# amathislab/BUCTD

Hardware: AMD Instinct MI355X
Metric: images/sec (train) BUCTD-CoAM-W48 384x288 (higher is better)
Workload: dtype f32 (3x3 convs: operands split exactly into 3 bf16 pieces, 6 bf16 MFMAs per product, fp32 accumulate - fp32-class); 1 GPU; BUCTD-CoAM-W48 (pose_hrnet_coam, ATT_MODULES [F,T,F,F], colored condition) 384x288 CrowdPose-14kpt full train step: fwd + JointsMSE + bwd + grad all-reduce + Adam + arg-max accuracy decode; global_batch=32, batch_per_gpu=32, input=N x 6 x 384 x 288 fp32, params=115581770, parallelism=dp1, hip_streams=4, conv_math=bf16x6, step_graph=False

## Files before the change

### buctd_amd/_C.py

```python
import ctypes as C
import os

import torch

_HERE = os.path.dirname(os.path.abspath(__file__))
LIB_PATH = os.path.join(_HERE, "lib", "libbuctd_hip.so")


class ConvDesc(C.Structure):
    _fields_ = [(n, C.c_int) for n in ("N", "H", "W", "Ci", "Co", "R", "S", "stride", "pad", "Ho", "Wo")]


class BasicBlockDesc(C.Structure):
    _fields_ = ([(n, C.c_int) for n in ("N", "H", "W", "C")] +
                [(n, C.c_void_p) for n in ("x", "w1_fwd", "w2_fwd", "w1_bwd", "w2_bwd", "gamma1", "beta1", "gamma2", "beta2",
                                           "running_mean1", "running_var1", "running_mean2", "running_var2")] +
                [(n, C.c_float) for n in ("eps1", "momentum1", "eps2", "momentum2")] +
                [(n, C.c_void_p) for n in ("z1", "z2", "y", "acc", "stat")])


class BasicBlockGrads(C.Structure):
    _fields_ = ([(n, C.c_void_p) for n in ("dy", "dz2", "dres", "dy1", "dz1", "dx", "dw1", "dw2", "dgamma1", "dbeta1",
                                           "dgamma2", "dbeta2")] +
                [(n, C.c_int) for n in ("acc_w1", "acc_w2", "acc_bn1", "acc_bn2")] +
# ... 2 lines not shown

class BnAccIn(C.Structure):
    _fields_ = [("acc", C.c_void_p), ("rows", C.c_long), ("eps", C.c_float), ("momentum", C.c_float),
                ("mean_out", C.c_void_p), ("invstd_out", C.c_void_p), ("running_mean", C.c_void_p),
                ("running_var", C.c_void_p)]


class C3Conv(C.Structure):
    _fields_ = ([(n, C.c_int) for n in ("N", "H", "W", "Ci", "Co")] +
                [(n, C.c_void_p) for n in ("x", "wprep", "residual")] + [("relu", C.c_int)] +
                [(n, C.c_void_p) for n in ("y", "stats_acc")] + [("in_bn", C.POINTER(BnAccIn))] +
                [(n, C.c_void_p) for n in ("in_gamma", "in_beta")] + [("in_relu", C.c_int)] +
                [(n, C.c_void_p) for n in ("bn_z", "bn_y", "bn_mean", "bn_invstd", "bn_gamma", "bn_beta", "bn_acc")])


class C3ConvEval(C.Structure):
    _fields_ = ([(n, C.c_int) for n in ("N", "H", "W", "Ci", "Co")] +
                [(n, C.c_void_p) for n in ("x", "wprep", "scale", "shift", "residual")] + [("relu", C.c_int), ("y", C.c_void_p)])


class BnApplyItem(C.Structure):
    _fields_ = [("z", C.c_void_p), ("st", BnAccIn), ("gamma", C.c_void_p), ("beta", C.c_void_p), ("residual", C.c_void_p),
                ("relu", C.c_int), ("y", C.c_void_p), ("rows", C.c_long), ("C", C.c_int)]


class BnBwdItem(C.Structure):
    _fields_ = ([(n, C.c_void_p) for n in ("dy", "y", "z", "mean", "invstd", "gamma", "beta")] +
                [("relu", C.c_int), ("rows", C.c_long), ("C", C.c_int)] +
                [(n, C.c_void_p) for n in ("dz", "dres", "dgamma", "dbeta")] +
                [("accumulate", C.c_int), ("acc", C.c_void_p), ("acc_ready", C.c_int)])


class Wg3Conv(C.Structure):
    _fields_ = ([(n, C.c_int) for n in ("N", "H", "W", "Ci", "Co")] +
                [(n, C.c_void_p) for n in ("x", "dy", "dw")] + [("accumulate", C.c_int)] +
                [(n, C.c_void_p) for n in ("x_mean", "x_invstd", "x_gamma", "x_beta")] + [("x_relu", C.c_int)] +
                [("workspace", C.c_void_p), ("workspace_bytes", C.c_size_t)])


class MhaArgs(C.Structure):
    _fields_ = ([(n, C.c_int) for n in ("B", "T", "h", "dh")] +
                [(n, C.c_void_p) for n in ("q", "k", "v")] + [(n, C.c_int) for n in ("ldq", "ldk", "ldv")] +
                [("out", C.c_void_p), ("ldo", C.c_int), ("lse", C.c_void_p), ("scale", C.c_float), ("p_drop", C.c_float),
                 ("dout", C.c_void_p), ("lddo", C.c_int)] +
                [(n, C.c_void_p) for n in ("dq", "dk", "dv")] + [(n, C.c_int) for n in ("lddq", "lddk", "lddv")])

# ... 108 lines not shown
    "buctd_conv3x3_wgrad_bf16x6_group_workgroups": (_I, [_I, C.POINTER(Wg3Conv)]),
    "buctd_stream_fork": (_I, [_P, _P]),
    "buctd_basic_branches_fwd_train": (_I, [_I, _I, C.POINTER(BasicBlockDesc), _P]),
    "buctd_basic_branches_bwd": (_I, [_I, _I, C.POINTER(BasicBlockDesc), C.POINTER(BasicBlockGrads), _P, _P]),
    "buctd_basic_chain_fwd_train": (_I, [_I, C.POINTER(BasicBlockDesc), _P]),
    "buctd_basic_chain_bwd": (_I, [_I, C.POINTER(BasicBlockDesc), C.POINTER(BasicBlockGrads), _P, _P]),
    "buctd_x6_image_dims": (_I, [_I, _I, _I, _P, _P]),
    "buctd_x6_image_bytes": (C.c_size_t, [_I, _I, _I]),
    "buctd_x6_image": (_I, [_P, _I, _I, _I, _L, _L, _I, _L, _L, _I, _P, _P]),
    "buctd_x6_gemm": (_I, [_I, _I, _I, _P, _P, _P, _I, _F, _P, _L, _I, _L, _P]),
    "buctd_add": (_I, [_P, _P, _P, _L, _I, _P]),
    "buctd_add_n": (_I, [C.POINTER(_P), _I, _P, _L, _P]),
    "buctd_mul": (_I, [_P, _P, _P, _L, _P]),
    "buctd_scale": (_I, [_P, _P, _F, _P, _L, _P]),
    "buctd_copy_channels": (_I, [_P, _L, _I, _I, _P, _I, _I, _I, _P]),
    "buctd_add_bcast": (_I, [_P, _P, _P, _L, _L, _P]),
    "buctd_relu_bwd": (_I, [_P, _P, _P, _L, _P]),
    "buctd_colsum_workspace": (_SZ, [_L, _I]),
    "buctd_colsum": (_I, [_P, _L, _I, _P, _I, _P, _SZ, _P]),
    "buctd_nchw_to_nhwc": (_I, [_P, _I, _I, _I, _I, _I, _I, _P, _P]),
    "buctd_nhwc_to_nchw": (_I, [_P, _I, _I, _I, _I, _P, _P]),
    "buctd_fuse_sum": (_I, [C.POINTER(_P), _PI, _I, _I, _I, _I, _I, _I, _P, _P]),
    "buctd_fuse_sum_bwd": (_I, [_P, _P, _I, _I, _I, _I, _I, _P, _P]),
    "buctd_resize_bilinear": (_I, [_P, _I, _I, _I, _I, _I, _I, _I, _I, _P, _P]),
    "buctd_maxpool3x3s2_fwd": (_I, [_P, _I, _I, _I, _I, _P, _P, _P]),
    "buctd_maxpool3x3s2_bwd": (_I, [_P, _P, _I, _I, _I, _I, _P, _P]),
    "buctd_softmax_dropout_fwd": (_I, [_P, _L, _I, _F, _F, _U64, _P, _P, _P]),
    "buctd_softmax_dropout_bwd": (_I, [_P, _P, _L, _I, _F, _F, _U64, _P, _P]),
    "buctd_softmax_dropout_fwd_dseed": (_I, [_P, _L, _I, _F, _F, _P, _P, _P, _P]),
    "buctd_softmax_dropout_bwd_dseed": (_I, [_P, _P, _L, _I, _F, _F, _P, _P, _P]),
    "buctd_dropout": (_I, [_P, _P, _L, _F, _U64, _P]),
    "buctd_dropout_dseed": (_I, [_P, _P, _L, _F, _P, _P]),
    "buctd_dropout_seed_fill": (_I, [_P, _I, _U64, _U64, _P]),
    "buctd_attn_smallqk_supported": (_I, [_I, _I, _I]),
    "buctd_attn_smallqk_fwd": (_I, [_I, _I, _I, _I, _P, _P, _P, _F, _F, _U64, _I, _P, _P, _P, _P]),
    "buctd_attn_smallqk_bwd": (_I, [_I, _I, _I, _I, _P, _P, _P, _P, _P, _P, _P, _F, _F, _U64, _I, _P, _P, _P, _P, _P]),
    "buctd_attn_smallqk_fwd_dseed": (_I, [_I, _I, _I, _I, _P, _P, _P, _F, _F, _P, _I, _P, _P, _P, _P]),
    "buctd_attn_smallqk_bwd_dseed": (_I, [_I, _I, _I, _I, _P, _P, _P, _P, _P, _P, _P, _F, _F, _P, _I, _P, _P, _P, _P, _P]),
    "buctd_layernorm_fwd": (_I, [_P, _P, _P, _L, _I, _F, _P, _P, _P, _P]),
    "buctd_add_layernorm_fwd": (_I, [_P, _P, _P, _P, _L, _I, _F, _P, _P, _P, _P, _P]),
    "buctd_layernorm_bwd_workspace": (_SZ, [_L, _I]),
    "buctd_layernorm_bwd": (_I, [_P, _P, _P, _P, _P, _L, _I, _P, _P, _P, _I, _P, _SZ, _P]),
    "buctd_joints_mse": (_I, [_P, _P, _P, _I, _I, _I, _P, _P, _F, _P, _SZ, _P]),
    "buctd_joints_ohkm_mse_workspace": (_SZ, [_I, _I]),
    "buctd_joints_ohkm_mse": (_I, [_P, _P, _P, _I, _I, _I, _I, _P, _P, _F, _P, _SZ, _P]),
    "buctd_argmax_decode": (_I, [_P, _I, _I, _I, _P, _P, _P, _P]),
# ... 102 lines not shown
```

### buctd_amd/csrc/bn.hip

```cpp
#include "common.h"
#include "../../include/buctd_hip.h"
#include "bn_acc.h"

#define STAT_ROWS 64

__global__ __launch_bounds__(256) void bn_stats_kernel(const float* __restrict__ z, long rows, int C,
                                                       float* __restrict__ part) {
  const long r0 = (long)blockIdx.x * STAT_ROWS;
  long r1 = r0 + STAT_ROWS;
  if (r1 > rows) r1 = rows;
  const int cnt = (int)(r1 - r0);
  for (int c = threadIdx.x; c < C; c += 256) {
    float s = 0.f;
    for (long r = r0; r < r1; ++r) s += z[r * C + c];
    const float mean = cnt > 0 ? s / (float)cnt : 0.f;
    float m2 = 0.f;
    for (long r = r0; r < r1; ++r) {
      const float d = z[r * C + c] - mean;
      m2 += d * d;
    }
    part[((long)blockIdx.x * C + c) * 2 + 0] = mean;
    part[((long)blockIdx.x * C + c) * 2 + 1] = m2;
  }
}

// ... 480 lines not shown
  const long total = rows * C;
  const float inv_rows = 1.0f / (float)rows;
  if (C % 4 == 0)
    hipLaunchKernelGGL(bn_bwd_apply_kernel<true>, dim3(stream_grid(total / 4)), dim3(256), 0, st, dy, y, z, mean,
                       invstd, gamma, beta, (const float*)s, relu, total, C, inv_rows, dz, dres);
  else
    hipLaunchKernelGGL(bn_bwd_apply_kernel<false>, dim3(stream_grid(total)), dim3(256), 0, st, dy, y, z, mean, invstd,
                       gamma, beta, (const float*)s, relu, total, C, inv_rows, dz, dres);
  BUCTD_CHECK_LAUNCH("buctd_bn_bwd_from_partials(apply)");
  return BUCTD_OK;
}

extern "C" int buctd_bn_fold(const float* gamma, const float* beta, const float* running_mean,
                             const float* running_var, float eps, int C, float* scale, float* shift, void* stream) {
  BUCTD_CHECK_ARG(gamma && beta && running_mean && running_var && scale && shift && C > 0,
                  "buctd_bn_fold: bad argument");
  hipLaunchKernelGGL(bn_fold_kernel, dim3(ceil_div(C, 256)), dim3(256), 0, (hipStream_t)stream, gamma, beta,
                     running_mean, running_var, eps, C, scale, shift);
  BUCTD_CHECK_LAUNCH("buctd_bn_fold");
  return BUCTD_OK;
}


#define BWD2_MAX_BLOCKS 1024

__global__ __launch_bounds__(256) void bn_bwd_reduce2_kernel(const float* __restrict__ dy, const float* __restrict__ y,
                                                             const float* __restrict__ z, const float* __restrict__ mean,
                                                             const float* __restrict__ invstd,
                                                             const float* __restrict__ gamma, const float* __restrict__ beta,
                                                             int relu, long rows, int C, long rows_per_block,
                                                             float* __restrict__ part) {
  __shared__ f32x4 sm[2][256];
  const int c4n = C >> 2;
  const int rl = 256 / c4n;
  const int tc = threadIdx.x % c4n, tr = threadIdx.x / c4n;
  const long r0 = (long)blockIdx.x * rows_per_block;
  long r1 = r0 + rows_per_block;
  if (r1 > rows) r1 = rows;
  f32x4 s1 = (f32x4){0.f, 0.f, 0.f, 0.f}, s2 = s1;
  if (tr < rl) {
    const f32x4 mu = reinterpret_cast<const f32x4*>(mean)[tc];
    const f32x4 is = reinterpret_cast<const f32x4*>(invstd)[tc];
    f32x4 sc = is, be = is;
    const bool rebuild = relu && !y;
    if (rebuild) {
      sc = is * reinterpret_cast<const f32x4*>(gamma)[tc];
      be = reinterpret_cast<const f32x4*>(beta)[tc];
    }
// ... 20 lines not shown
      }
#pragma unroll
      for (int u = 0; u < 4; ++u) body(g[u], zz[u], yy[u]);
    }
    for (; r < r1; r += step) {
      const long o = r * c4n + tc;
      const f32x4 zz = reinterpret_cast<const f32x4*>(z)[o];
      body(reinterpret_cast<const f32x4*>(dy)[o], zz, (relu && y) ? reinterpret_cast<const f32x4*>(y)[o] : zz);
    }
  }
  sm[0][threadIdx.x] = s1;
  sm[1][threadIdx.x] = s2;
  __syncthreads();
  if (tr == 0) {
    for (int k = 1; k < rl; ++k) {
      s1 += sm[0][k * c4n + tc];
      s2 += sm[1][k * c4n + tc];
    }
    reinterpret_cast<f32x4*>(part + ((long)blockIdx.x * 2 + 0) * C)[tc] = s1;
    reinterpret_cast<f32x4*>(part + ((long)blockIdx.x * 2 + 1) * C)[tc] = s2;
  }
}

static long bwd2_blocks(long rows, long* rows_per_block) {
  long rpb = (rows + BWD2_MAX_BLOCKS - 1) / BWD2_MAX_BLOCKS;
  if (rpb < 64) rpb = 64;
  *rows_per_block = rpb;
  return (rows + rpb - 1) / rpb;
}


static int acc_grid(long n4, int per_cu = 8) {
  long b = (n4 + 256 * 4 - 1) / (256 * 4);
  if (b > 256 * per_cu) b = 256 * per_cu;
  if (b < 1) b = 1;
  return (int)b;
}

struct BnApplyArgs {
  const float* z;
  BnAccFwd a;
  const float* gamma;
  const float* beta;
  const float* res;
  int relu;
  float* y;
  long total;
  int C;
};
__device__ __forceinline__ void bn_apply_acc_body(const BnApplyArgs& p, unsigned bid, unsigned nblk, unsigned char* lds_raw) {
  const float* __restrict__ z = p.z;
  const float* __restrict__ res = p.res;
  float* __restrict__ y = p.y;
  const BnAccFwd& a = p.a;
  const int C = p.C, relu = p.relu;
  long long* wsum = reinterpret_cast<long long*>(lds_raw);
  float* tab = reinterpret_cast<float*>(lds_raw + (size_t)BNACC_WORDS * C * sizeof(long long));
  const long n4 = p.total >> 2;
  const long step = (long)nblk * 256;
  long i = (long)bid * 256 + threadIdx.x;
// ... 422 lines not shown
```

### buctd_amd/models/hrnet_common.py

```python
import logging
import os

import torch

from .. import nn
from .. import ops

BN_MOMENTUM = 0.1
logger = logging.getLogger(__name__)


def conv3x3(in_planes, out_planes, stride=1):
    return nn.Conv2d(in_planes, out_planes, kernel_size=3, stride=stride, padding=1, bias=False)


class BasicBlock(nn.Module):
    expansion = 1

    def __init__(self, inplanes, planes, stride=1, downsample=None):
        super().__init__()
        self.conv1 = conv3x3(inplanes, planes, stride)
        self.bn1 = nn.BatchNorm2d(planes, momentum=BN_MOMENTUM)
        self.relu = nn.ReLU(inplace=True)
        self.conv2 = conv3x3(planes, planes)
# ... 164 lines not shown
                       and m.bn1.running_mean is not None and m.bn2.running_mean is not None for m in br):
                return None
            chains.append([_block_params(m) for m in br])
        xs = [x[i] for i in range(self.num_branches)]
        if not ops.eval_branches_ok(xs, chains):
            return None
        return ops.basic_branches_eval(xs, chains)

    def forward(self, x):
        if self.num_branches == 1:
            return [self.branches[0](x[0])]
        xs = self._branches_grouped(x)
        if xs is None:
            xs = self._branches_grouped_eval(x)
        if xs is None:
            xs = ops.fork_join([lambda i=i: self.branches[i](x[i]) for i in range(self.num_branches)],
                               [x[i] for i in range(self.num_branches)])
        rows = list(enumerate(self.fuse_layers))
        fan = len(rows) > 1 and torch.is_grad_enabled() and any(t.requires_grad for t in xs)
        xr = [ops.FanOut.apply(xs[j], len(rows)) if fan and xs[j].is_cuda else [xs[j]] * len(rows)
              for j in range(self.num_branches)]

        def fuse_row(i, row):
            terms, shifts = [], []
            for j in range(self.num_branches):
                if j == i:
                    terms.append(xr[j][i])
                    shifts.append(0)
                elif j > i:
                    terms.append(row[j](xr[j][i]))
                    shifts.append(j - i)
                else:
                    terms.append(row[j](xr[j][i]))
                    shifts.append(0)
            return ops.FuseSum.apply(tuple(shifts), True, *terms)

        return ops.fork_join([lambda i=i, row=row: fuse_row(i, row) for i, row in rows], [xs for _ in rows], tag=1)


def make_transition_layer(pre, cur):
    layers = []
    for i in range(len(cur)):
        if i < len(pre):
            if cur[i] != pre[i]:
                layers.append(nn.ConvBN(nn.Conv2d(pre[i], cur[i], 3, 1, 1, bias=False), nn.BatchNorm2d(cur[i]),
                                        nn.ReLU(inplace=True)))
            else:
                layers.append(None)
        else:
            steps = []
            for j in range(i + 1 - len(pre)):
                cin = pre[-1]
                cout = cur[i] if j == i - len(pre) else cin
                steps.append(nn.ConvBN(nn.Conv2d(cin, cout, 3, 2, 1, bias=False), nn.BatchNorm2d(cout),
                                       nn.ReLU(inplace=True)))
            layers.append(nn.Chain(*steps))
    return nn.ModuleList(layers)

# ... 89 lines not shown
```

### buctd_amd/ops.py

```python
import ctypes as C
import math
import weakref

import torch

from . import _C
from ._C import ConvDesc, MatmulDesc, check, lib, ptr, stream_ptr

_capture = {"on": False, "events": set(), "allow_seeds": False, "seed_table": None, "seed_draws": 0}
_SEED_TABLE_SLOTS = 1024


def capturing():
    return _capture["on"]


def _new_event(stream=None):
    ev = torch.cuda.Event()
    ev.record(stream) if stream is not None else ev.record()
    if _capture["on"]:
        _capture["events"].add(id(ev))
        _capture.setdefault("keep", []).append(ev)
    return ev

# ... 1876 lines not shown
class FuseSum(torch.autograd.Function):

    @staticmethod
    def forward(ctx, shifts, relu, *terms):
        out = fuse_sum(list(terms), list(shifts), relu)
        ctx.shifts, ctx.relu = shifts, relu
        ctx.save_for_backward(out if relu else None)
        return out

    @staticmethod
    def backward(ctx, dy):
        (y,) = ctx.saved_tensors
        dy = _contig(dy)
        cache = {}
        grads = []
        for j, s in enumerate(ctx.shifts):
            if not ctx.needs_input_grad[2 + j]:
                grads.append(None)
                continue
            if s not in cache:
                cache[s] = fuse_sum_bwd(dy, y, s) if s > 0 or ctx.relu else dy
            grads.append(cache[s])
        return (None, None, *grads)


class AddN(torch.autograd.Function):

    @staticmethod
    def forward(ctx, a, b, c):
        out = add(a, b)
        if c is not None:
            out = add(out, c, out=out)
        ctx.n = 3 if c is not None else 2
        return out

    @staticmethod
    def backward(ctx, dy):
        return dy, dy, (dy if ctx.n == 3 else None)


def add_n(terms):
    acc = terms[0]
    k = 1
    while k < len(terms):
        group = [acc] + list(terms[k:k + 3])
        k += 3
# ... 391 lines not shown
```

### include/buctd_hip.h

```cpp
#ifndef BUCTD_HIP_H
#define BUCTD_HIP_H
#include <stddef.h>
#include <stdint.h>

#ifdef __cplusplus
extern "C" {
#endif

int buctd_version(void);
const char* buctd_last_error(void);

typedef struct {
  int N, H, W, Ci;
  int Co, R, S;
  int stride, pad;
  int Ho, Wo;
} buctd_conv_desc;

int buctd_conv2d_fwd_thin(const buctd_conv_desc* d);
int buctd_conv2d_fwd(const buctd_conv_desc* d, const float* x, const float* w, const float* bias,
                     const float* scale, const float* shift, const float* residual, int relu, float* y,
                     float* stats_partials, void* stream);
int buctd_conv2d_dgrad(const buctd_conv_desc* d, const float* dy, const float* w, const float* bias, float* dx,
                       float* stats_partials, void* stream);
// ... 167 lines not shown
  int acc_ready;
} buctd_bn_bwd_item;
int buctd_bn_bwd_acc_group(int n, const buctd_bn_bwd_item* items, void* stream);
int buctd_bn_fold(const float* gamma, const float* beta, const float* running_mean, const float* running_var,
                  float eps, int C, float* scale, float* shift, void* stream);

int buctd_add(const float* a, const float* b, float* out, long n, int relu, void* stream);
int buctd_add_n(const float* const* terms, int n, float* out, long count, void* stream);
int buctd_mul(const float* a, const float* b, float* out, long n, void* stream);
int buctd_scale(const float* x, const float* dev_scalar, float alpha, float* out, long n, void* stream);
int buctd_copy_channels(const float* src, long rows, int Cs, int cs0, float* dst, int Cd, int cd0, int Cc,
                        void* stream);
int buctd_add_bcast(const float* a, const float* v, float* out, long batch, long n, void* stream);
int buctd_relu_bwd(const float* dy, const float* y, float* dx, long n, void* stream);
size_t buctd_colsum_workspace(long rows, int C);
int buctd_colsum(const float* x, long rows, int C, float* out, int accumulate, void* workspace,
                 size_t workspace_bytes, void* stream);
int buctd_nchw_to_nhwc(const float* x, int N, int Ctot, int c0, int Cc, int H, int W, float* y, void* stream);
int buctd_nhwc_to_nchw(const float* x, int N, int C, int H, int W, float* y, void* stream);
int buctd_fuse_sum(const float* const* terms, const int* shifts, int nterms, int N, int H, int W, int C, int relu,
                   float* out, void* stream);
int buctd_fuse_sum_bwd(const float* dy, const float* y, int shift, int N, int H, int W, int C, float* g,
                       void* stream);
int buctd_resize_bilinear(const float* x, int N, int Ctot, int c0, int Cc, int H, int W, int Ho, int Wo, float* y,
                          void* stream);
int buctd_maxpool3x3s2_fwd(const float* x, int N, int H, int W, int C, float* y, int32_t* idx, void* stream);
int buctd_maxpool3x3s2_bwd(const float* dy, const int32_t* idx, int N, int H, int W, int C, float* dx,
                           void* stream);

int buctd_softmax_dropout_fwd(const float* s, long rows, int L, float scale, float p_drop, uint64_t seed, float* p,
                              float* pd, void* stream);
int buctd_softmax_dropout_bwd(const float* dpd, const float* p, long rows, int L, float scale, float p_drop,
                              uint64_t seed, float* ds, void* stream);
int buctd_softmax_dropout_fwd_dseed(const float* s, long rows, int L, float scale, float p_drop, const uint64_t* seed,
                                    float* p, float* pd, void* stream);
int buctd_softmax_dropout_bwd_dseed(const float* dpd, const float* p, long rows, int L, float scale, float p_drop,
                                    const uint64_t* seed, float* ds, void* stream);
int buctd_attn_smallqk_supported(int T, int R4, int C);
int buctd_attn_smallqk_fwd(int B, int T, int R4, int C, const float* q, const float* k, const float* v, float scale,
                           float p_drop, uint64_t seed, int bf16x3, float* out, float* m, float* linv, void* stream);
int buctd_attn_smallqk_bwd(int B, int T, int R4, int C, const float* q, const float* k, const float* v,
                           const float* o, const float* dout, const float* m, const float* linv, float scale,
                           float p_drop, uint64_t seed, int bf16x3, float* dq, float* dk, float* dv,
                           float* dvec_workspace, void* stream);
int buctd_attn_smallqk_fwd_dseed(int B, int T, int R4, int C, const float* q, const float* k, const float* v, float scale,
                                 float p_drop, const uint64_t* seed, int bf16x3, float* out, float* m, float* linv,
// ... 273 lines not shown
```

Baseline: 490.7 images/s.

## Fuse HRNet fuse-layer BN apply, upsample-sum and ReLU into per-row kernels

Adds a FuseRow autograd op and three HIP kernels that fold the batch-norm apply of every branch term, the nearest-neighbour upsample by shift, the sum and the ReLU into one forward launch. The backward path forms the upsampled/ReLU-masked gradient and computes the BN reductions and input gradients for all terms in batched reduce and apply launches. This replaces the earlier per-term bn_apply + fuse_sum forward and the fuse_sum_bwd + per-term BN backward. It is meant to cut kernel launches and intermediate activation round trips to memory. In exchange the kernels recompute the upsampled gradient gather per term, hold the stat tables in LDS, and fall back to the old path when fuse_row_ok rejects the inputs.

```diff
diff --git a/buctd_amd/_C.py b/buctd_amd/_C.py
--- a/buctd_amd/_C.py
+++ b/buctd_amd/_C.py
@@ -48,6 +48,12 @@
 class BnApplyItem(C.Structure):
     _fields_ = [("z", C.c_void_p), ("st", BnAccIn), ("gamma", C.c_void_p), ("beta", C.c_void_p), ("residual", C.c_void_p),
                 ("relu", C.c_int), ("y", C.c_void_p), ("rows", C.c_long), ("C", C.c_int)]
+
+
+class FuseTerm(C.Structure):
+    _fields_ = ([("z", C.c_void_p), ("shift", C.c_int), ("has_bn", C.c_int), ("st", BnAccIn)] +
+                [(n, C.c_void_p) for n in ("gamma", "beta", "mean", "invstd", "dz", "dgamma", "dbeta")] +
+                [("accumulate", C.c_int), ("acc", C.c_void_p)])
 
 
 class BnBwdItem(C.Structure):
@@ -202,6 +208,9 @@
     "buctd_nhwc_to_nchw": (_I, [_P, _I, _I, _I, _I, _P, _P]),
     "buctd_fuse_sum": (_I, [C.POINTER(_P), _PI, _I, _I, _I, _I, _I, _I, _P, _P]),
     "buctd_fuse_sum_bwd": (_I, [_P, _P, _I, _I, _I, _I, _I, _P, _P]),
+    "buctd_fuse_row_fwd": (_I, [_I] * 5 + [C.POINTER(FuseTerm), _I, _P, _P]),
+    "buctd_fuse_row_bwd_reduce": (_I, [_I] * 5 + [C.POINTER(FuseTerm), _P, _P, _P]),
+    "buctd_fuse_row_bwd_apply": (_I, [_I] * 5 + [C.POINTER(FuseTerm), _P, _P, _P]),
     "buctd_resize_bilinear": (_I, [_P, _I, _I, _I, _I, _I, _I, _I, _I, _P, _P]),
     "buctd_maxpool3x3s2_fwd": (_I, [_P, _I, _I, _I, _I, _P, _P, _P]),
     "buctd_maxpool3x3s2_bwd": (_I, [_P, _P, _I, _I, _I, _I, _P, _P]),
diff --git a/buctd_amd/csrc/bn.hip b/buctd_amd/csrc/bn.hip
--- a/buctd_amd/csrc/bn.hip
+++ b/buctd_amd/csrc/bn.hip
@@ -1,6 +1,7 @@
 #include "common.h"
 #include "../../include/buctd_hip.h"
 #include "bn_acc.h"
+#include "bn_tiling.h"
 
 #define STAT_ROWS 64
 
@@ -527,8 +528,6 @@
 }
 
 
-#define BWD2_MAX_BLOCKS 1024
-
 __global__ __launch_bounds__(256) void bn_bwd_reduce2_kernel(const float* __restrict__ dy, const float* __restrict__ y,
                                                              const float* __restrict__ z, const float* __restrict__ mean,
                                                              const float* __restrict__ invstd,
@@ -595,20 +594,10 @@
   }
 }
 
-static long bwd2_blocks(long rows, long* rows_per_block) {
-  long rpb = (rows + BWD2_MAX_BLOCKS - 1) / BWD2_MAX_BLOCKS;
-  if (rpb < 64) rpb = 64;
-  *rows_per_block = rpb;
-  return (rows + rpb - 1) / rpb;
-}
-
-
-static int acc_grid(long n4, int per_cu = 8) {
-  long b = (n4 + 256 * 4 - 1) / (256 * 4);
-  if (b > 256 * per_cu) b = 256 * per_cu;
-  if (b < 1) b = 1;
-  return (int)b;
-}
+static long bwd2_blocks(long rows, long* rows_per_block) { return bn_bwd2_blocks(rows, rows_per_block); }
+
+
+static int acc_grid(long n4, int per_cu = 8) { return bn_acc_grid(n4, per_cu); }
 
 struct BnApplyArgs {
   const float* z;
diff --git a/buctd_amd/csrc/bn_tiling.h b/buctd_amd/csrc/bn_tiling.h
--- /dev/null
+++ b/buctd_amd/csrc/bn_tiling.h
@@ -0,0 +1,17 @@
+#pragma once
+
+#define BWD2_MAX_BLOCKS 1024
+
+static inline long bn_bwd2_blocks(long rows, long* rows_per_block) {
+  long rpb = (rows + BWD2_MAX_BLOCKS - 1) / BWD2_MAX_BLOCKS;
+  if (rpb < 64) rpb = 64;
+  *rows_per_block = rpb;
+  return (rows + rpb - 1) / rpb;
+}
+
+static inline int bn_acc_grid(long n4, int per_cu = 8) {
+  long b = (n4 + 256 * 4 - 1) / (256 * 4);
+  if (b > 256 * per_cu) b = 256 * per_cu;
+  if (b < 1) b = 1;
+  return (int)b;
+}
diff --git a/buctd_amd/csrc/fuse_row.hip b/buctd_amd/csrc/fuse_row.hip
--- /dev/null
+++ b/buctd_amd/csrc/fuse_row.hip
@@ -0,0 +1,373 @@
+#include "common.h"
+#include "bn_acc.h"
+#include "bn_tiling.h"
+#include "../../include/buctd_hip.h"
+
+#define FR_MAX 4
+
+struct FrTerm {
+  const float* z;
+  int shift, has_bn;
+  BnAccFwd a;
+  const float* gamma;
+  const float* beta;
+  const float* mean;
+  const float* invstd;
+  float* dz;
+  float* dgamma;
+  float* dbeta;
+  int accumulate;
+  long long* acc;
+  long rows;
+  long rows_per_block;
+  float inv_rows;
+};
+struct FrArgs {
+  FrTerm t[FR_MAX];
+  int nterms;
+  int N, H, W, C;
+  int relu;
+  const float* dy;
+  const float* y;
+  float* yo;
+  unsigned first[FR_MAX + 1];
+};
+
+__global__ __launch_bounds__(256, 8) void fuse_row_fwd_kernel(FrArgs p_) {
+  extern __shared__ __attribute__((aligned(16))) unsigned char lds_raw[];
+  const FrArgs& p = *(const FrArgs*)__builtin_amdgcn_kernarg_segment_ptr();
+  const int C = p.C, C4 = C >> 2, H = p.H, W = p.W, nterms = p.nterms;
+  long long* wsum = reinterpret_cast<long long*>(lds_raw);
+  float* tabs = reinterpret_cast<float*>(lds_raw + (size_t)BNACC_WORDS * C * sizeof(long long));
+  for (int j = 0; j < nterms; ++j) {
+    const FrTerm& t = p.t[j];
+    if (!t.has_bn) continue;
+    const BnAccFwd& a = t.a;
+    float* tab = tabs + (size_t)j * 3 * C;
+    bnacc_gather_lds(a.acc, C, wsum);
+    for (int c = threadIdx.x; c < C; c += 256) {
+      double s1, s2;
+      bnacc_read_lds(wsum, C, c, &s1, &s2);
+      const BnFwdStat st = bnacc_fwd_stat_sums(s1, s2, a.rows, a.eps);
+      tab[c] = st.mean;
+      tab[C + c] = st.invstd * t.gamma[c];
+      tab[2 * C + c] = t.beta[c];
+      if (blockIdx.x == 0) {
+        a.mean_out[c] = st.mean;
+        a.invstd_out[c] = st.invstd;
+        if (a.rmean) bnacc_running(st, a.rows, a.momentum, a.rmean, a.rvar, c);
+      }
+    }
+    __syncthreads();
+  }
+  const long total = (long)p.N * H * W * C4;
+  const long step = (long)gridDim.x * 256;
+  float* __restrict__ out = p.yo;
+  for (long i = (long)blockIdx.x * 256 + threadIdx.x; i < total; i += step) {
+    const int c4 = (int)(i % C4);
+    long pix = i / C4;
+    const int w = (int)(pix % W);
+    pix /= W;
+    const int h = (int)(pix % H);
+    const int n = (int)(pix / H);
+    f32x4 zz[FR_MAX];
+#pragma unroll
+    for (int j = 0; j < FR_MAX; ++j) {
+      if (j < nterms) {
+        const int s = p.t[j].shift;
+        const int hs = H >> s, ws = W >> s;
+        const long o = (((long)n * hs + (h >> s)) * ws + (w >> s)) * C4 + c4;
+        zz[j] = reinterpret_cast<const f32x4*>(p.t[j].z)[o];
+      }
+    }
+    f32x4 v = (f32x4){0.f, 0.f, 0.f, 0.f};
+#pragma unroll
+    for (int j = 0; j < FR_MAX; ++j) {
+      if (j < nterms) {
+        f32x4 o = zz[j];
+        if (p.t[j].has_bn) {
+          const float* tab = tabs + (size_t)j * 3 * C + c4 * 4;
+          const f32x4 mu = *reinterpret_cast<const f32x4*>(tab);
+          const f32x4 sc = *reinterpret_cast<const f32x4*>(tab + C);
+          const f32x4 be = *reinterpret_cast<const f32x4*>(tab + 2 * C);
+#pragma unroll
+          for (int j4 = 0; j4 < 4; ++j4) o[j4] = (zz[j][j4] - mu[j4]) * sc[j4] + be[j4];
+        }
+        v += o;
+      }
+    }
+    if (p.relu) {
+#pragma unroll
+      for (int j4 = 0; j4 < 4; ++j4) v[j4] = fmaxf(v[j4], 0.f);
+    }
+    reinterpret_cast<f32x4*>(out)[i] = v;
+  }
+}
+
+template <int CH>
+__device__ __forceinline__ f32x4 fr_form_g(const float* __restrict__ dy, const float* __restrict__ y, int s, int H, int W,
+                                           int C4, long r, int c4) {
+  const int hs = H >> s, ws = W >> s, f = 1 << s;
+  const int w = (int)(r % ws);
+  const long q = r / ws;
+  const int h = (int)(q % hs);
+  const long n = q / hs;
+  f32x4 acc = (f32x4){0.f, 0.f, 0.f, 0.f};
+  for (int dh = 0; dh < f; ++dh) {
+    const long o0 = ((n * H + h * f + dh) * W + w * f) * C4 + c4;
+    for (int dw0 = 0; dw0 < f; dw0 += CH) {
+      f32x4 d[CH], yy[CH];
+#pragma unroll
+      for (int u = 0; u < CH; ++u) {
+        if (dw0 + u < f) {
+          d[u] = reinterpret_cast<const f32x4*>(dy)[o0 + (long)(dw0 + u) * C4];
+          if (y) yy[u] = reinterpret_cast<const f32x4*>(y)[o0 + (long)(dw0 + u) * C4];
+        }
+      }
+#pragma unroll
+      for (int u = 0; u < CH; ++u) {
+        if (dw0 + u < f) {
+          if (y) {
+#pragma unroll
+            for (int j = 0; j < 4; ++j)
+              if (!(yy[u][j] > 0.f)) d[u][j] = 0.f;
+          }
+          acc += d[u];
+        }
+      }
+    }
+  }
+  return acc;
+}
+
+__device__ __forceinline__ int fr_find(const FrArgs& p, unsigned* bid, unsigned* nblk) {
+  int k = 0;
+  while (k + 1 < p.nterms && blockIdx.x >= p.first[k + 1]) ++k;
+  *bid = blockIdx.x - p.first[k];
+  *nblk = p.first[k + 1] - p.first[k];
+  return k;
+}
+
+__global__ __launch_bounds__(256) void fuse_row_bwd_reduce_kernel(FrArgs p_) {
+  __shared__ f32x4 sm[2][256];
+  const FrArgs& p = *(const FrArgs*)__builtin_amdgcn_kernarg_segment_ptr();
+  unsigned bid, nblk;
+  const FrTerm& t = p.t[fr_find(p, &bid, &nblk)];
+  const float* __restrict__ z = t.z;
+  const int C = p.C, c4n = C >> 2;
+  const int rl = 256 / c4n;
+  const int tc = threadIdx.x % c4n, tr = threadIdx.x / c4n;
+  const long r0 = (long)bid * t.rows_per_block;
+  long r1 = r0 + t.rows_per_block;
+  if (r1 > t.rows) r1 = t.rows;
+  f32x4 s1 = (f32x4){0.f, 0.f, 0.f, 0.f}, s2 = s1;
+  if (tr < rl) {
+    const f32x4 mu = reinterpret_cast<const f32x4*>(t.mean)[tc];
+    const f32x4 is = reinterpret_cast<const f32x4*>(t.invstd)[tc];
+    const int s = t.shift;
+    const long step = rl;
+    long r = r0 + tr;
+    if (s == 0) {
+      for (; r + 3 * step < r1; r += 4 * step) {
+        f32x4 g[4], zz[4];
+#pragma unroll
+        for (int u = 0; u < 4; ++u) {
+          g[u] = fr_form_g<1>(p.dy, p.y, 0, p.H, p.W, c4n, r + u * step, tc);
+          zz[u] = reinterpret_cast<const f32x4*>(z)[(r + u * step) * c4n + tc];
+        }
+#pragma unroll
+        for (int u = 0; u < 4; ++u) {
+          s1 += g[u];
+          s2 += g[u] * (zz[u] - mu) * is;
+        }
+      }
+    }
+    for (; r < r1; r += step) {
+      const f32x4 zz = reinterpret_cast<const f32x4*>(z)[r * c4n + tc];
+      const f32x4 g = fr_form_g<8>(p.dy, p.y, s, p.H, p.W, c4n, r, tc);
+      if (s > 0) reinterpret_cast<f32x4*>(t.dz)[r * c4n + tc] = g;
+      s1 += g;
+      s2 += g * (zz - mu) * is;
+    }
+  }
+  sm[0][threadIdx.x] = s1;
+  sm[1][threadIdx.x] = s2;
+  __syncthreads();
+  if (tr == 0) {
+    for (int k = 1; k < rl; ++k) {
+      s1 += sm[0][k * c4n + tc];
+      s2 += sm[1][k * c4n + tc];
+    }
+    sm[0][tc] = s1;
+    sm[1][tc] = s2;
+  }
+  __syncthreads();
+  const unsigned shard = bnacc_shard();
+  for (int c = threadIdx.x; c < C; c += 256)
+    bnacc_add(t.acc, C, shard, c, (double)reinterpret_cast<const float*>(&sm[0][0])[c], (double)reinterpret_cast<const float*>(&sm[1][0])[c]);
+}
+
+__global__ __launch_bounds__(256, 6) void fuse_row_bwd_apply_kernel(FrArgs p_) {
+  extern __shared__ __attribute__((aligned(16))) unsigned char lds_raw[];
+  const FrArgs& p = *(const FrArgs*)__builtin_amdgcn_kernarg_segment_ptr();
+  unsigned bid, nblk;
+  const FrTerm& t = p.t[fr_find(p, &bid, &nblk)];
+  const int C = p.C, C4 = C >> 2, s = t.shift;
+  const long n4 = t.rows * C4;
+  const long step = (long)nblk * 256;
+  float* __restrict__ dz = t.dz;
+  if (!t.has_bn) {
+    for (long i = (long)bid * 256 + threadIdx.x; i < n4; i += step)
+      reinterpret_cast<f32x4*>(dz)[i] = fr_form_g<4>(p.dy, p.y, s, p.H, p.W, C4, i / C4, (int)(i % C4));
+    return;
+  }
+  const float* __restrict__ z = t.z;
+  long long* wsum = reinterpret_cast<long long*>(lds_raw);
+  float* tab = reinterpret_cast<float*>(lds_raw + (size_t)BNACC_WORDS * C * sizeof(long long));
+  const float inv_rows = t.inv_rows;
+  bnacc_gather_lds(t.acc, C, wsum);
+  for (int c = threadIdx.x; c < C; c += 256) {
+    double s1, s2;
+    bnacc_read_lds(wsum, C, c, &s1, &s2);
+    tab[c] = t.mean[c];
+    tab[C + c] = t.invstd[c];
+    tab[2 * C + c] = t.gamma[c];
+    tab[3 * C + c] = (float)s1;
+    tab[4 * C + c] = (float)s2;
+    if (bid == 0) {
+      if (t.dbeta) t.dbeta[c] = t.accumulate ? t.dbeta[c] + (float)s1 : (float)s1;
+      if (t.dgamma) t.dgamma[c] = t.accumulate ? t.dgamma[c] + (float)s2 : (float)s2;
+    }
+  }
+  __syncthreads();
+  for (long i = (long)bid * 256 + threadIdx.x; i < n4; i += step) {
+    const int c4 = (int)(i % C4);
+    const f32x4 zz = reinterpret_cast<const f32x4*>(z)[i];
+    const f32x4 g = s > 0 ? reinterpret_cast<const f32x4*>(dz)[i] : fr_form_g<1>(p.dy, p.y, 0, p.H, p.W, C4, i / C4, c4);
+    const float* tb = tab + c4 * 4;
+    const f32x4 mu = *reinterpret_cast<const f32x4*>(tb);
+    const f32x4 is = *reinterpret_cast<const f32x4*>(tb + C);
+    const f32x4 ga = *reinterpret_cast<const f32x4*>(tb + 2 * C);
+    const f32x4 s1 = *reinterpret_cast<const f32x4*>(tb + 3 * C);
+    const f32x4 s2 = *reinterpret_cast<const f32x4*>(tb + 4 * C);
+    f32x4 o;
+#pragma unroll
+    for (int j4 = 0; j4 < 4; ++j4) {
+      const float zh = (zz[j4] - mu[j4]) * is[j4];
+      o[j4] = ga[j4] * is[j4] * (g[j4] - s1[j4] * inv_rows - zh * s2[j4] * inv_rows);
+    }
+    reinterpret_cast<f32x4*>(dz)[i] = o;
+  }
+}
+
+static int fr_fill(const char* who, int N, int H, int W, int C, int nterms, const buctd_fuse_term* terms, FrArgs& a) {
+  BUCTD_CHECK_ARG(terms && nterms >= 1 && nterms <= FR_MAX, "%s: 1..%d terms", who, FR_MAX);
+  BUCTD_CHECK_ARG(N > 0 && H > 0 && W > 0 && C > 0 && C % 4 == 0 && C <= 1024, "%s: C must be a multiple of 4, <= 1024", who);
+  a.nterms = nterms;
+  a.N = N; a.H = H; a.W = W; a.C = C;
+  a.relu = 0;
+  a.dy = a.y = nullptr;
+  a.yo = nullptr;
+  for (int j = 0; j <= FR_MAX; ++j) a.first[j] = 0;
+  for (int j = 0; j < FR_MAX; ++j) {
+    FrTerm& t = a.t[j];
+    t = FrTerm{};
+    if (j >= nterms) continue;
+    const buctd_fuse_term& u = terms[j];
+    BUCTD_CHECK_ARG(u.z != nullptr && u.shift >= 0 && u.shift <= 5, "%s: bad term %d", who, j);
+    BUCTD_CHECK_ARG((H >> u.shift) << u.shift == H && (W >> u.shift) << u.shift == W,
+                    "%s: H/W not divisible by 2^shift for term %d", who, j);
+    t.z = u.z; t.shift = u.shift; t.has_bn = u.has_bn != 0;
+    t.rows = (long)N * (H >> u.shift) * (W >> u.shift);
+    t.gamma = u.gamma; t.beta = u.beta; t.mean = u.mean; t.invstd = u.invstd;
+    t.dz = u.dz; t.dgamma = u.dgamma; t.dbeta = u.dbeta; t.accumulate = u.accumulate; t.acc = (long long*)u.acc;
+    t.inv_rows = 1.0f / (float)t.rows;
+    bn_bwd2_blocks(t.rows, &t.rows_per_block);
+  }
+  return BUCTD_OK;
+}
+
+extern "C" int buctd_fuse_row_fwd(int N, int H, int W, int C, int nterms, const buctd_fuse_term* terms, int relu, float* y,
+                                  void* stream) {
+  FrArgs a;
+  if (const int rc = fr_fill("buctd_fuse_row_fwd", N, H, W, C, nterms, terms, a)) return rc;
+  BUCTD_CHECK_ARG(y, "buctd_fuse_row_fwd: no output");
+  for (int j = 0; j < nterms; ++j) {
+    if (!a.t[j].has_bn) continue;
+    const buctd_bn_acc_in& st = terms[j].st;
+    BUCTD_CHECK_ARG(st.acc && st.rows > 0 && st.mean_out && st.invstd_out && (st.running_mean == nullptr) == (st.running_var == nullptr),
+                    "buctd_fuse_row_fwd: statistics accumulator, rows, mean_out and invstd_out are required; running_mean/var go together");
+    BUCTD_CHECK_ARG(a.t[j].gamma && a.t[j].beta, "buctd_fuse_row_fwd: term %d has no gamma / beta", j);
+    BUCTD_CHECK_ARG(st.rows == a.t[j].rows, "buctd_fuse_row_fwd: the statistics cover %ld rows, the tensor has %ld", st.rows, a.t[j].rows);
+    BnAccFwd& f = a.t[j].a;
+    f.acc = (const long long*)st.acc; f.rows = (double)st.rows; f.eps = st.eps; f.momentum = st.momentum;
+    f.mean_out = st.mean_out; f.invstd_out = st.invstd_out; f.rmean = st.running_mean; f.rvar = st.running_var;
+  }
+  a.relu = relu;
+  a.yo = y;
+  const long total = (long)N * H * W * (C / 4);
+  const size_t lds = (size_t)(BNACC_WORDS * 8 + 3 * 4 * nterms) * C;
+  if (lds > 64 * 1024) {
+    static unsigned char attr_done[BUCTD_MAX_DEVICES] = {0};
+    if (const int rc = buctd_raise_lds_limit(reinterpret_cast<const void*>(fuse_row_fwd_kernel), 160 * 1024, attr_done, "buctd_fuse_row_fwd"))
+      return rc;
+  }
+  hipLaunchKernelGGL(fuse_row_fwd_kernel, dim3(bn_acc_grid(total)), dim3(256), lds, (hipStream_t)stream, a);
+  BUCTD_CHECK_LAUNCH("buctd_fuse_row_fwd");
+  return BUCTD_OK;
+}
+
+static int fr_bwd_check(const char* who, int nterms, const FrArgs& a, const float* dy) {
+  BUCTD_CHECK_ARG(dy, "%s: no output gradient", who);
+  for (int j = 0; j < nterms; ++j) {
+    const FrTerm& t = a.t[j];
+    if (t.has_bn)
+      BUCTD_CHECK_ARG(t.mean && t.invstd && t.gamma && t.dz && t.acc, "%s: term %d needs mean, invstd, gamma, dz and acc", who, j);
+  }
+  return BUCTD_OK;
+}
+
+extern "C" int buctd_fuse_row_bwd_reduce(int N, int H, int W, int C, int nterms, const buctd_fuse_term* terms, const float* dy,
+                                         const float* y, void* stream) {
+  FrArgs a, g;
+  if (const int rc = fr_fill("buctd_fuse_row_bwd_reduce", N, H, W, C, nterms, terms, a)) return rc;
+  if (const int rc = fr_bwd_check("buctd_fuse_row_bwd_reduce", nterms, a, dy)) return rc;
+  g = a;
+  g.nterms = 0;
+  g.dy = dy; g.y = y;
+  for (int sh = 5; sh >= 0; --sh)
+  for (int j = 0; j < nterms; ++j) {
+    if (!a.t[j].has_bn || a.t[j].shift != sh) continue;
+    g.t[g.nterms] = a.t[j];
+    long rpb;
+    g.first[g.nterms + 1] = g.first[g.nterms] + (unsigned)bn_bwd2_blocks(a.t[j].rows, &rpb);
+    ++g.nterms;
+  }
+  if (g.nterms == 0) return BUCTD_OK;
+  for (int k = g.nterms; k < FR_MAX; ++k) g.first[k + 1] = g.first[g.nterms];
+  hipLaunchKernelGGL(fuse_row_bwd_reduce_kernel, dim3(g.first[g.nterms]), dim3(256), 0, (hipStream_t)stream, g);
+  BUCTD_CHECK_LAUNCH("buctd_fuse_row_bwd_reduce");
+  return BUCTD_OK;
+}
+
+extern "C" int buctd_fuse_row_bwd_apply(int N, int H, int W, int C, int nterms, const buctd_fuse_term* terms, const float* dy,
+                                        const float* y, void* stream) {
+  FrArgs a, g;
+  if (const int rc = fr_fill("buctd_fuse_row_bwd_apply", N, H, W, C, nterms, terms, a)) return rc;
+  if (const int rc = fr_bwd_check("buctd_fuse_row_bwd_apply", nterms, a, dy)) return rc;
+  g = a;
+  g.nterms = 0;
+  g.dy = dy; g.y = y;
+  for (int j = 0; j < nterms; ++j) {
+    if (!a.t[j].has_bn && !a.t[j].dz) continue;
+    g.t[g.nterms] = a.t[j];
+    g.first[g.nterms + 1] = g.first[g.nterms] + (unsigned)bn_acc_grid(a.t[j].rows * (C / 4), 6);
+    ++g.nterms;
+  }
+  if (g.nterms == 0) return BUCTD_OK;
+  for (int k = g.nterms; k < FR_MAX; ++k) g.first[k + 1] = g.first[g.nterms];
+  hipLaunchKernelGGL(fuse_row_bwd_apply_kernel, dim3(g.first[g.nterms]), dim3(256), (size_t)(BNACC_WORDS * 8 + 5 * 4) * C,
+                     (hipStream_t)stream, g);
+  BUCTD_CHECK_LAUNCH("buctd_fuse_row_bwd_apply");
+  return BUCTD_OK;
+}
diff --git a/buctd_amd/models/hrnet_common.py b/buctd_amd/models/hrnet_common.py
--- a/buctd_amd/models/hrnet_common.py
+++ b/buctd_amd/models/hrnet_common.py
@@ -210,18 +210,13 @@
               for j in range(self.num_branches)]
 
         def fuse_row(i, row):
-            terms, shifts = [], []
+            terms = []
             for j in range(self.num_branches):
-                if j == i:
-                    terms.append(xr[j][i])
-                    shifts.append(0)
-                elif j > i:
-                    terms.append(row[j](xr[j][i]))
-                    shifts.append(j - i)
-                else:
-                    terms.append(row[j](xr[j][i]))
-                    shifts.append(0)
-            return ops.FuseSum.apply(tuple(shifts), True, *terms)
+                steps = [] if j == i else [row[j]] if j > i else list(row[j])
+                for m in steps:
+                    nn._as_channels_last_(m[0].weight)
+                terms.append((max(j - i, 0), [(m[0], m[1], m._relu) for m in steps]))
+            return ops.fuse_row([xr[j][i] for j in range(self.num_branches)], terms)[0]
 
         return ops.fork_join([lambda i=i, row=row: fuse_row(i, row) for i, row in rows], [xs for _ in rows], tag=1)
 
diff --git a/buctd_amd/ops.py b/buctd_amd/ops.py
--- a/buctd_amd/ops.py
+++ b/buctd_amd/ops.py
@@ -1922,6 +1922,188 @@
                 cache[s] = fuse_sum_bwd(dy, y, s) if s > 0 or ctx.relu else dy
             grads.append(cache[s])
         return (None, None, *grads)
+
+
+_FUSE_ROWS = True
+FUSE_ROW_MAX_TERMS = 4
+
+
+def _fuse_row_acc_route(x_shape, conv):
+    stride, pad = conv._geom()
+    d = conv_desc(tuple(x_shape), _wshape(conv.weight), stride, pad)
+    ok = _conv_math["mode"] == "bf16x6" and conv.bias is None and (_bf16x3_ok(d) or _gconv_ok(d, 0))
+    return ok, (d.N, d.Ho, d.Wo, d.Co)
+
+
+def fuse_row_ok(xs, terms):
+    if not (_FUSE_ROWS and torch.is_grad_enabled() and 1 < len(terms) <= FUSE_ROW_MAX_TERMS and len(xs) == len(terms)):
+        return False
+    for x, (shift, steps) in zip(xs, terms):
+        if not (x.is_cuda and x.dtype == torch.float32 and x.dim() == 4 and x.is_contiguous()):
+            return False
+        shape = tuple(x.shape)
+        for k, (conv, bn, relu) in enumerate(steps):
+            last = k == len(steps) - 1
+            if not (isinstance(conv, torch.nn.Conv2d) and bn.training and (not last or not relu)):
+                return False
+            acc, shape = _fuse_row_acc_route(shape, conv)
+            if last and not acc:
+                return False
+        if not (shape[-1] % 4 == 0 and bn_acc_ok(shape[-1])):
+            return False
+    return True
+
+
+def _fuse_term_array(specs):
+    arr = (_C.FuseTerm * len(specs))()
+    for t, sp in zip(arr, specs):
+        for k, v in sp.items():
+            setattr(t, k, v)
+    return arr
+
+
+def fuse_row_fwd(zs, shifts, bnins, relu=True):
+    base = zs[shifts.index(0)]
+    N, H, W, Cn = base.shape
+    y = torch.empty_like(base)
+    specs = []
+    for z, s, b in zip(zs, shifts, bnins):
+        sp = {"z": z.data_ptr(), "shift": s, "has_bn": int(b is not None)}
+        if b is not None:
+            sp.update(st=b.struct(), gamma=b.gamma.data_ptr(), beta=b.beta.data_ptr())
+        specs.append(sp)
+    check(lib().buctd_fuse_row_fwd(N, H, W, Cn, len(zs), _fuse_term_array(specs), int(bool(relu)), ptr(y), stream_ptr()),
+          "fuse_row_fwd")
+    return y
+
+
+def fuse_row_bwd(dy, y, zs, shifts, bns, want_plain):
+    N, H, W, Cn = dy.shape
+    specs, outs, keep = [], [], []
+    for z, s, b, want in zip(zs, shifts, bns, want_plain):
+        sp = {"z": z.data_ptr(), "shift": s, "has_bn": int(b is not None)}
+        dz = (torch.empty((N, H >> s, W >> s, Cn), dtype=torch.float32, device=dy.device)
+              if (b is not None or want) else None)
+        if dz is not None:
+            sp["dz"] = dz.data_ptr()
+        if b is not None:
+            mean, invstd, gamma, dgamma, dbeta, accumulate = b
+            acc = AccRef(Cn, z.device)
+            keep.append(acc)
+            sp.update(mean=mean.data_ptr(), invstd=invstd.data_ptr(), gamma=gamma.data_ptr(), dgamma=dgamma.data_ptr(),
+                      dbeta=dbeta.data_ptr(), accumulate=int(accumulate), acc=acc.ptr)
+        specs.append(sp)
+        outs.append(dz)
+    arr = _fuse_term_array(specs)
+    check(lib().buctd_fuse_row_bwd_reduce(N, H, W, Cn, len(zs), arr, ptr(dy), ptr(y), stream_ptr()), "fuse_row_bwd_reduce")
+    check(lib().buctd_fuse_row_bwd_apply(N, H, W, Cn, len(zs), arr, ptr(dy), ptr(y), stream_ptr()), "fuse_row_bwd_apply")
+    return outs
+
+
+class FuseRow(torch.autograd.Function):
+
+    @staticmethod
+    def forward(ctx, terms, relu, *xs):
+        subs, zs, shifts, bnins, lasts = [], [], [], [], []
+        for j, (shift, steps) in enumerate(terms):
+            x = xs[j]
+            for k, (conv, bn, act) in enumerate(steps[:-1]):
+                c = _SubCtx(ctx.needs_input_grad[2 + j] if k == 0 else True)
+                s, p = conv._geom()
+                x = ConvBnAct.forward(c, x, conv.weight, conv.bias, bn, None, act, s, p, True, None)
+                subs.append(c)
+            shifts.append(shift)
+            if not steps:
+                zs.append(x)
+                bnins.append(None)
+                lasts.append(None)
+                continue
+            conv, bn, _ = steps[-1]
+            s, p = conv._geom()
+            z, acc, info = conv_fwd(x, conv.weight, None, s, p, stats="acc")
+            if info[0] != "acc":
+                raise _C.BuctdHipError("FuseRow: the last convolution of term %d left no statistics accumulator (fuse_row_ok "
+                                       "decides the route before the node is built)" % j)
+            zs.append(z)
+            bnins.append(BnAccInput(acc, z.numel() // z.shape[-1], bn, True, relu=False))
+            lasts.append((x, z))
+        y = fuse_row_fwd(zs, shifts, bnins, relu)
+        for (_, steps), b in zip(terms, bnins):
+            if b is not None and b.rm is not None:
+                _count_batch(steps[-1][1])
+        ctx.terms, ctx.relu, ctx.shifts, ctx.nsub = terms, relu, shifts, len(subs)
+        tail = _SubCtx()
+        tail.save_for_backward(*[t for la, b in zip(lasts, bnins) if la is not None for t in (la[0], la[1], b.mean, b.invstd)],
+                               y if relu else None)
+        ctx.sub = subs + [tail]
+        _pack_subs(ctx, ctx.sub)
+        return y
+
+    @staticmethod
+    def backward(ctx, dy):
+        terms, relu, shifts = ctx.terms, ctx.relu, ctx.shifts
+        _unpack_subs(ctx, ctx.sub)
+        subs, tail = ctx.sub[:-1], ctx.sub[-1]
+        saved = list(tail.saved_tensors)
+        y = saved.pop()
+        dy = _contig(dy)
+        zs, bns, want_plain, xin = [], [], [], []
+        it = iter(saved)
+        for j, (shift, steps) in enumerate(terms):
+            if not steps:
+                zs.append(dy)
+                bns.append(None)
+                want_plain.append(bool(ctx.needs_input_grad[2 + j]) and (relu or shift > 0))
+                xin.append(None)
+                continue
+            x, z, mean, invstd = next(it), next(it), next(it), next(it)
+            bn = steps[-1][1]
+            dgamma, acc_g = grad_target(bn.weight)
+            dbeta, acc_b = grad_target(bn.bias)
+            assert acc_g == acc_b
+            zs.append(z)
+            bns.append((mean, invstd, bn.weight, dgamma, dbeta, acc_g))
+            want_plain.append(False)
+            xin.append(x)
+        dzs = fuse_row_bwd(dy, y, zs, shifts, bns, want_plain)
+        grads = [None] * len(terms)
+        first_sub = []
+        n = 0
+        for _, steps in terms:
+            first_sub.append(n)
+            n += max(len(steps) - 1, 0)
+        for j in range(len(terms) - 1, -1, -1):
+            shift, steps = terms[j]
+            if not steps:
+                if ctx.needs_input_grad[2 + j]:
+                    grads[j] = dzs[j] if want_plain[j] else dy
+                continue
+            conv, bn, _ = steps[-1]
+            s, p = conv._geom()
+            dz, x = dzs[j], xin[j]
+            need = ctx.needs_input_grad[2 + j] if len(steps) == 1 else True
+            g = conv_dgrad(dz, conv.weight, tuple(x.shape), s, p) if need else None
+            dw, acc_w = grad_target(conv.weight)
+            conv_wgrad_async(x, dz, conv.weight, s, p, dw, acc_w)
+            grad_done(bn.weight, bn.bias, conv.weight, None)
+            for k in range(len(steps) - 2, -1, -1):
+                g = ConvBnAct.backward(subs[first_sub[j] + k], g)[0]
+            grads[j] = g
+        for c in ctx.sub:
+            c.saved_tensors = ()
+        return (None, None, *grads)
+
+
+def fuse_row(xs, terms, relu=True):
+    if fuse_row_ok(xs, terms):
+        return FuseRow.apply(terms, relu, *xs), True
+    ts = []
+    for x, (_, steps) in zip(xs, terms):
+        for conv, bn, act in steps:
+            s, p = conv._geom()
+            x = ConvBnAct.apply(x, conv.weight, conv.bias, bn, None, act, s, p, bn.training, None)
+        ts.append(x)
+    return FuseSum.apply(tuple(s for s, _ in terms), relu, *ts), False
 
 
 class AddN(torch.autograd.Function):
diff --git a/include/buctd_hip.h b/include/buctd_hip.h
--- a/include/buctd_hip.h
+++ b/include/buctd_hip.h
@@ -213,6 +213,24 @@
                    float* out, void* stream);
 int buctd_fuse_sum_bwd(const float* dy, const float* y, int shift, int N, int H, int W, int C, float* g,
                        void* stream);
+typedef struct {
+  const float* z;
+  int shift;
+  int has_bn;
+  buctd_bn_acc_in st;
+  const float *gamma, *beta;
+  const float *mean, *invstd;
+  float* dz;
+  float *dgamma, *dbeta;
+  int accumulate;
+  void* acc;
+} buctd_fuse_term;
+int buctd_fuse_row_fwd(int N, int H, int W, int C, int nterms, const buctd_fuse_term* terms, int relu, float* y,
+                       void* stream);
+int buctd_fuse_row_bwd_reduce(int N, int H, int W, int C, int nterms, const buctd_fuse_term* terms, const float* dy,
+                              const float* y, void* stream);
+int buctd_fuse_row_bwd_apply(int N, int H, int W, int C, int nterms, const buctd_fuse_term* terms, const float* dy,
+                             const float* y, void* stream);
 int buctd_resize_bilinear(const float* x, int N, int Ctot, int c0, int Cc, int H, int W, int Ho, int Wo, float* y,
                           void* stream);
 int buctd_maxpool3x3s2_fwd(const float* x, int N, int H, int W, int C, float* y, int32_t* idx, void* stream);
diff --git a/scratch/fuse_rows_profile.py b/scratch/fuse_rows_profile.py
--- /dev/null
+++ b/scratch/fuse_rows_profile.py
@@ -0,0 +1,104 @@
+import bisect, collections, csv, sys
+
+FAMILIES = ("bn_apply_acc_kernel", "bn_bwd_reduce_acc_kernel", "bn_bwd_apply_acc_kernel", "fuse_sum_kernel", "fuse_sum_bwd_kernel",
+            "fuse_row_fwd_kernel", "fuse_row_bwd_reduce_kernel", "fuse_row_bwd_apply_kernel")
+
+
+def family(name):
+    for f in FAMILIES:
+        if name.startswith(f + "("):
+            return f
+    return None
+
+
+def load(path):
+    rows = list(csv.DictReader(open(path)))
+    ks = sorted(((int(r["Start_Timestamp"]), int(r["End_Timestamp"]), r["Kernel_Name"], r.get("Queue_Id", "0"), int(r["Grid_Size_X"]))
+                 for r in rows), key=lambda t: t[0])
+    adam = [i for i, k in enumerate(ks) if k[2].startswith("adam_kernel")]
+    return [ks[a + 1:b + 1] for a, b in zip(adam[:-1], adam[1:])]
+
+
+def per_step(steps):
+    steps = steps[-8:]
+    n, t = collections.Counter(), collections.Counter()
+    for st in steps:
+        for s, e, name, q, grid in st:
+            f = family(name)
+            if f:
+                n[(f, grid)] += 1
+                t[(f, grid)] += e - s
+    k = float(len(steps))
+    launches = sum(len(st) for st in steps) / k
+    wall = sum(max(x[1] for x in st) - st[0][0] for st in steps) / k / 1e6
+    return {key: (n[key] / k, t[key] / k / 1e6) for key in n}, launches, wall
+
+
+def chain(st):
+    by_end = sorted(range(len(st)), key=lambda i: st[i][1])
+    ends = [st[i][1] for i in by_end]
+    cur = max(range(len(st)), key=lambda i: st[i][1])
+    on = collections.Counter()
+    total = 0
+    while True:
+        s, e, name, q, grid = st[cur]
+        total += e - s
+        f = family(name)
+        if f:
+            on[(f, grid)] += (e - s) / 1e6
+        j = bisect.bisect_right(ends, s + 1000) - 1
+        while j >= 0 and by_end[j] == cur:
+            j -= 1
+        if j < 0 or cur == 0:
+            break
+        cur = by_end[j]
+    return on, total / 1e6
+
+
+def report(out, title, stats, launches, wall, on, chain_ms, share):
+    with open(out, "w") as fh:
+        fh.write(title + "\n")
+        fh.write(f"whole step: {launches:.0f} kernel launches, {wall:.2f} ms wall under the tracer; last-arrival chain of step 1: {chain_ms:.2f} ms in kernels\n")
+        fh.write("fuse-row part per step (launches, summed kernel ms, on-chain ms)   |   rest of the network (launches, ms)   kernel\n")
+        tl = tm = tc = 0.0
+        for f in FAMILIES:
+            keys = [k for k in stats if k[0] == f]
+            if not keys:
+                continue
+            fl = sum(stats[k][0] * share(k) for k in keys)
+            fm = sum(stats[k][1] * share(k) for k in keys)
+            fc = sum(on.get(k, 0.0) * share(k) for k in keys)
+            rl = sum(stats[k][0] for k in keys) - fl
+            rm = sum(stats[k][1] for k in keys) - fm
+            tl, tm, tc = tl + fl, tm + fm, tc + fc
+            fh.write(f"  {fl:6.1f} {fm:7.3f} {fc:7.3f}   |   {rl:6.1f} {rm:7.3f}   {f}\n")
+        fh.write(f"  {tl:6.1f} {tm:7.3f} {tc:7.3f}   total of the fuse-row part\n")
+        fh.write("by grid size (workgroups x 256 threads), fuse-row share of the launches:\n")
+        for k in sorted(stats):
+            if share(k) > 0:
+                fh.write(f"  {k[0]:28s} grid {k[1] // 256:5d}: {stats[k][0]:5.1f} launches, {stats[k][1] * 1e3 / max(stats[k][0], 1e-9):6.1f} us each, share {share(k):.2f}\n")
+
+
+before, after = load(sys.argv[1]), load(sys.argv[2])
+sb, lb, wb = per_step(before)
+sa, la, wa = per_step(after)
+NEW = ("fuse_row_fwd_kernel", "fuse_row_bwd_reduce_kernel", "fuse_row_bwd_apply_kernel")
+
+
+def share_before(k):
+    if k[0] in ("fuse_sum_kernel", "fuse_sum_bwd_kernel"):
+        return 1.0
+    gone = sb[k][0] - sa.get(k, (0.0, 0.0))[0]
+    return max(0.0, min(1.0, gone / sb[k][0]))
+
+
+def share_after(k):
+    return 1.0 if k[0] in NEW or k[0] in ("fuse_sum_kernel", "fuse_sum_bwd_kernel") else 0.0
+
+
+ob, cb = chain(before[1])
+oa, ca = chain(after[1])
+report(sys.argv[3], "Fuse rows BEFORE (parent build: bn_apply_acc per term + fuse_sum; fuse_sum_bwd + bn_bwd reduce / apply per term)",
+       sb, lb, wb, ob, cb, share_before)
+report(sys.argv[4], "Fuse rows AFTER (ops.FuseRow: fuse_row_fwd, fuse_row_bwd_reduce, fuse_row_bwd_apply per row)",
+       sa, la, wa, oa, ca, share_after)
```

Measured after the change: 491.0 images/s, median of 3. No clear change (+0.1%).
